# oarodriguez/PhD-QMCLib

Measured on AMD Instinct MI355X. Metric: walker-steps/sec, higher is better.
Workload: dtype f64

## Files before the change

### phd_qmclib_amd/csrc/qmc_device.h

```cpp
#pragma once

#include <hip/hip_runtime.h>
#include <stdint.h>

#include "qmc_math.h"

#define QMC_PI 3.141592653589793238462643383279502884

#define QMC_NSEC 32
#define QMC_SEC_COPIES 1024
#define QMC_NDIAG 4
#if defined(QMC_TIMING)
#define QMC_SECTION(name) qmc_stamp(m, qmc_sec_id(name))
#define QMC_SECTION_PHASE(off) qmc_stamp_phase(off)
#elif defined(QMC_CUTS)
#define QMC_SECTION(name)                                                     \
    do {                                                                      \
        if (m.sec_cut == qmc_sec_id(name) + QMC_SEC_OFF)                      \
            __builtin_amdgcn_endpgm();                                        \
    } while (0)
#define QMC_SECTION_PHASE(off) do { } while (0)
#elif defined(QMC_SECTIONS)
#define QMC_SECTION(name) asm volatile("; SECTION " name)
#define QMC_SECTION_PHASE(off) do { } while (0)
// ... 74 lines not shown
    unsigned long long last[4];
    int cur[4], phase[4];
};
__device__ __forceinline__ QmcStampState &qmc_stamp_state()
{
    __shared__ QmcStampState st;
    return st;
}
__device__ __forceinline__ void qmc_stamp_phase(int off)
{
    if ((threadIdx.x & 63) == 0) qmc_stamp_state().phase[threadIdx.x >> 6] = off;
}
__device__ __forceinline__ void qmc_stamp(const DevModel &m, int id)
{
    const unsigned long long t = __builtin_readcyclecounter();
    if ((threadIdx.x & 63) == 0 && m.sec_prof) {
        QmcStampState &st = qmc_stamp_state();
        const int w = threadIdx.x >> 6;
        if (id != 0) {
            const int c = (st.cur[w] & (QMC_NSEC - 1)) +
                          2 * QMC_NSEC * (blockIdx.x & (QMC_SEC_COPIES - 1));
            atomicAdd(&m.sec_prof[c], t - st.last[w]);
            atomicAdd(&m.sec_prof[QMC_NSEC + c], 1ull);
        } else {
            st.phase[w] = 0;
        }
        st.cur[w] = id + st.phase[w];
        st.last[w] = t;
    }
}
#endif

#define OB_DEG 7
#define OB_ROW 16

enum { STREAM_VMC_MOVE = 0, STREAM_VMC_ACCEPT = 1, STREAM_DMC_BRANCH = 2,
       STREAM_DMC_DIFFUSE = 3 };

__device__ __forceinline__ void philox4x32_10(uint32_t (&c)[4], uint32_t k0,
                                              uint32_t k1)
{
#pragma unroll
    for (int r = 0; r < 10; ++r) {
        uint64_t p0 = (uint64_t)0xD2511F53u * c[0];
        uint64_t p1 = (uint64_t)0xCD9E8D57u * c[2];
        uint32_t n0 = (uint32_t)(p1 >> 32) ^ c[1] ^ k0;
        uint32_t n2 = (uint32_t)(p0 >> 32) ^ c[3] ^ k1;
        c[0] = n0; c[1] = (uint32_t)p1; c[2] = n2; c[3] = (uint32_t)p0;
        k0 += 0x9E3779B9u; k1 += 0xBB67AE85u;
    }
}

__device__ __forceinline__ double u53(uint32_t hi, uint32_t lo)
{
    const double a = (double)(hi >> 5);
    const double b = (double)(lo >> 6);
    return fma(a, 0x1p-27, b * 0x1p-53);
}

__device__ __forceinline__ void philox_uniform2(uint64_t seed, uint32_t slot,
                                                uint32_t step, uint32_t index,
                                                uint32_t stream, double &u0,
                                                double &u1)
{
    uint32_t c[4] = { slot, step, index, stream };
    philox4x32_10(c, (uint32_t)seed, (uint32_t)(seed >> 32));
    u0 = u53(c[0], c[1]);
    u1 = u53(c[2], c[3]);
}

__device__ __forceinline__ void philox2x32_10(uint32_t &c0, uint32_t &c1,
                                              uint32_t k)
{
#pragma unroll
    for (int r = 0; r < 10; ++r) {
        const uint64_t p = (uint64_t)0xD256D193u * c0;
        const uint32_t n0 = (uint32_t)(p >> 32) ^ k ^ c1;
        c1 = (uint32_t)p;
        c0 = n0;
        k += 0x9E3779B9u;
    }
}

__device__ __forceinline__ void vmc_move_block(uint64_t seed, uint32_t slot,
                                               uint32_t step, uint32_t index,
                                               uint32_t &w0, uint32_t &w1)
{
    uint32_t key = (uint32_t)seed ^ ((uint32_t)(seed >> 32) * 0x85EBCA6Bu);
    key += (step >> 26) * 0x632BE5ABu + (slot >> 28) * 0xC2B2AE35u;
    w0 = ((step & 0x3FFFFFFu) << 6) | ((slot >> 22) & 0x3Fu);
    w1 = ((slot & 0x3FFFFFu) << 10) | (index & 0x3FFu);
    philox2x32_10(w0, w1, key);
}

__device__ __forceinline__ double vmc_move_unit(uint32_t w0)
{
    return fma((double)w0, 0x1p-32, 0x1p-33 - 0.5);
}

__device__ __forceinline__ void normal2_from_uniforms(double u0, double u1,
                                                      double &g0, double &g1)
{
    double r = fast_sqrt(fmax(-2.0 * log_pos(1.0 - u0), 1e-300));
    double s, c;
    sincos_halfpi(4.0 * u1, s, c);
    g0 = r * c;
    g1 = r * s;
}

__device__ __forceinline__ void philox_normal2(uint64_t seed, uint32_t slot,
                                               uint32_t step, uint32_t index,
                                               uint32_t stream, double &g0,
                                               double &g1)
{
    double u0, u1;
    philox_uniform2(seed, slot, step, index, stream, u0, u1);
    normal2_from_uniforms(u0, u1, g0, g1);
}

__device__ __forceinline__ void normal2_from_words(uint32_t w0, uint32_t w1,
                                                   double &g0, double &g1)
{
    const double u0 = fma((double)w0, 0x1p-32, 0x1p-33);
    const double u1 = fma((double)w1, 0x1p-32, 0x1p-33);
    const double r = fast_sqrt(-2.0 * log_pos(u0));
    double s, c;
    sincos_halfpi(4.0 * u1, s, c);
    g0 = r * c;
    g1 = r * s;
}

__device__ __forceinline__ void dmc_normal2(uint64_t seed, uint32_t slot,
                                            uint32_t step2, uint32_t index,
                                            double &g0, double &g1)
{
    uint32_t key = (uint32_t)seed ^ ((uint32_t)(seed >> 32) * 0x85EBCA6Bu);
    key += 0x27D4EB2Fu;
    key += (step2 >> 26) * 0x632BE5ABu + (slot >> 28) * 0xC2B2AE35u;
    uint32_t w0 = ((step2 & 0x3FFFFFFu) << 6) | ((slot >> 22) & 0x3Fu);
    uint32_t w1 = ((slot & 0x3FFFFFu) << 10) | (index & 0x3FFu);
    philox2x32_10(w0, w1, key);
    normal2_from_words(w0, w1, g0, g1);
}

__device__ __forceinline__ double wrap_box(double z, double L)
{
    double zw = (z < 0.0) ? z + L : (z >= L) ? z - L : z;
    const bool far = z < -L || z >= 2.0 * L;
    if (__builtin_expect(__ballot(far) != 0ull, 0)) {
        const double r = fma(-L, floor(z / L), z);
        zw = far ? (r < 0.0 ? r + L : r) : zw;
    }
    return zw;
}

template <int G, int P>
struct SlotMap {
    static constexpr bool CONSECUTIVE = (G == 64) && (P >= 2);
};

template <int G, bool PAD>
__device__ __forceinline__ int lanes_in_use(const DevModel &m)
{
    return PAD ? m.ge : G;
}

template <int G, int P, bool PAD>
__device__ __forceinline__ int walker_n(const DevModel &m)
{
    return PAD ? m.n : G * P;
}

template <int G, int P, bool PAD>
__device__ __forceinline__ int lane_particle(const DevModel &m, int gl, int p)
{
    if (SlotMap<G, P>::CONSECUTIVE) return P * gl + p;
    if (!PAD) return gl + G * p;
    const int ge = m.ge;
    return gl < ge ? gl + ge * p : m.n;
}

template <int N>
__device__ __forceinline__ double row_ror_f64(double v)
{
    const int lo = __builtin_amdgcn_update_dpp(0, __double2loint(v), 0x120 + N,
                                               0xf, 0xf, false);
    const int hi = __builtin_amdgcn_update_dpp(0, __double2hiint(v), 0x120 + N,
                                               0xf, 0xf, false);
    return __hiloint2double(hi, lo);
}

template <int G>
__device__ __forceinline__ double group_sum(double v)
{
    static_assert(G >= 16, "lane groups are 16, 32 or 64 lanes");
    v += row_ror_f64<8>(v);
    v += row_ror_f64<4>(v);
    v += row_ror_f64<2>(v);
    v += row_ror_f64<1>(v);
#pragma unroll
    for (int m = 16; m < G; m <<= 1)
        v += __shfl_xor(v, m, 64);
    return v;
}

__device__ __forceinline__ double wave_sum_mfma(double v)
{
    const double r = __builtin_amdgcn_mfma_f64_4x4x4f64(v, 1.0, 0.0, 0, 0, 0);
    double t = __builtin_amdgcn_mfma_f64_4x4x4f64(r, 1.0, 0.0, 0, 0, 0);
    t += row_ror_f64<4>(t);
    t += row_ror_f64<8>(t);
    return t;
}

template <int G, int P>
__device__ __forceinline__ void resort_step(double (&z)[P], int (&lab)[P],
                                            int gl, unsigned parity, int n,
                                            double L, double half_L,
                                            int ge = G)
{
    const int lane = threadIdx.x & 63, base = lane - gl;
    int pg = (parity & 1u) ? ((gl & 1) ? gl + 1 : gl - 1) : (gl ^ 1);
    const bool wrap_hi = pg >= ge, wrap_lo = pg < 0;
    if (wrap_hi) pg = 0;
    if (wrap_lo) pg = ge - 1;
    double z0[P]; int l0[P];
#pragma unroll
    for (int a = 0; a < P; ++a) { z0[a] = z[a]; l0[a] = lab[a]; }
#pragma unroll
    for (int a = 0; a < P; ++a) {
        const int want = wrap_hi ? (a + 1) % P : (wrap_lo ? (a + P - 1) % P : a);
        double zp = 0.0; int lp = 0;
#pragma unroll
        for (int b = 0; b < P; ++b) {
            double zz = __shfl(z0[b], base + pg, 64);
            int ll = __shfl(l0[b], base + pg, 64);
            if (b == want) { zp = zz; lp = ll; }
        }
        const bool valid = gl < ge && (gl + ge * a) < n &&
                           (pg + ge * want) < n;
        const bool lower = wrap_hi ? true : (wrap_lo ? false : gl < pg);
        double d = lower ? zp - z0[a] : z0[a] - zp;
        if (d > half_L) d -= L;
        if (d < -half_L) d += L;
        if (valid && d < 0.0) { z[a] = zp; lab[a] = lp; }
    }
}

template <int G>
__device__ __forceinline__ void resort_linear(double &z, int &lab, int gl,
                                              unsigned parity, int ge)
{
    const int lane = threadIdx.x & 63, base = lane - gl;
    const int pg = (parity & 1u) ? ((gl & 1) ? gl + 1 : gl - 1) : (gl ^ 1);
    const bool has = gl < ge && pg >= 0 && pg < ge;
    const int src = base + (has ? pg : gl);
    const double zp = __shfl(z, src, 64);
    const int lp = __shfl(lab, src, 64);
    const bool take = has && ((gl < pg) ? zp < z : zp > z);
    if (take) { z = zp; lab = lp; }
}

template <int G>
__device__ __forceinline__ int group_ror1_b32(int x)
{
    static_assert(G == 64 || G == 16, "a DPP rotation exists for 16 and 64 lanes");
    if (G == 64) return __builtin_amdgcn_update_dpp(x, x, 0x13C, 0xf, 0xf, false);
    return __builtin_amdgcn_update_dpp(x, x, 0x121, 0xf, 0xf, false);
}
template <int G>
__device__ __forceinline__ double group_ror1(double v)
{
    return __hiloint2double(group_ror1_b32<G>(__double2hiint(v)),
                            group_ror1_b32<G>(__double2loint(v)));
}
template <int G>
__device__ __forceinline__ float group_ror1(float v)
{
    return __int_as_float(group_ror1_b32<G>(__float_as_int(v)));
}

__device__ __forceinline__ double readlane_f64(double v, int lane)
{
    const int lo = __builtin_amdgcn_readlane(__double2loint(v), lane);
    const int hi = __builtin_amdgcn_readlane(__double2hiint(v), lane);
    return __hiloint2double(hi, lo);
}

__device__ __forceinline__ void anchor_seam(double &z, int &lab,
                                            int ge )
{
    const int lane = threadIdx.x & 63;
    const double z0 = readlane_f64(z, 0), zl = readlane_f64(z, ge - 1);
    if (zl < z0) {
        const double z1 = readlane_f64(z, 1), zl1 = readlane_f64(z, ge - 2);
        int src = lane;
        if (zl < z1) {
            if (lane < ge) src = lane == 0 ? ge - 1 : lane - 1;
        } else if (z0 > zl1) {
            if (lane < ge) src = lane == ge - 1 ? 0 : lane + 1;
        }
        z = __shfl(z, src, 64);
        lab = __shfl(lab, src, 64);
    }
}

// ... 969 lines not shown
```

### phd_qmclib_amd/csrc/qmc_kernels.h

```cpp
#pragma once

#include "qmc_device.h"
#include "qmc_sorted64.h"
#include "qmc_sorted128.h"

static constexpr int BLOCK = 256;

static constexpr int BLOCK64 = 64;
template <int G>
struct WalkBlock {
    static constexpr int N = (G == 64) ? BLOCK64 : BLOCK;
};

template <int GPB>
__device__ __forceinline__ long long walker_of_block(unsigned b, int grp)
{
    if (GPB == 1)
        return ((long long)(b >> 7) << 7) + ((b & 7u) << 4) + ((b & 127u) >> 3);
    return (long long)b * GPB + grp;
}

template <int G, int P, bool PAD, bool ZC, bool DMC = false>
struct StepLds {
    static constexpr int NROWS =
        DMC ? SortedCot<false, true, false>::ROWS : 5;
    static constexpr int SORTED =
        (G == 64 && P == 2 && !ZC)   ? NROWS * SortedRows<128>::ROW
        : (G == 64 && P == 1 && !ZC) ? NROWS * SortedRows<64>::ROW
                                     : 0;
    static constexpr int GENERAL = GroupLds<G, P, ZC>::DOUBLES;
    static constexpr int DOUBLES = SORTED > GENERAL ? SORTED : GENERAL;
};

__device__ __forceinline__ long long qmc_uniform(long long v)
{
    const int lo = __builtin_amdgcn_readfirstlane((int)v);
    const int hi = __builtin_amdgcn_readfirstlane((int)(v >> 32));
    return ((long long)hi << 32) | (unsigned int)lo;
}
__device__ __forceinline__ int qmc_opaque(int v)
{
    asm volatile("" : "+v"(v));
    return v;
}
__device__ __forceinline__ double qmc_uniform_f64(double v)
{
    return __longlong_as_double(qmc_uniform(__double_as_longlong(v)));
}
__device__ __forceinline__ double qmc_lane_f64(double v, int k)
{
    const long long b = __double_as_longlong(v);
    const int lo = __builtin_amdgcn_readlane((int)b, k);
    const int hi = __builtin_amdgcn_readlane((int)(b >> 32), k);
    return __longlong_as_double(((long long)hi << 32) | (unsigned int)lo);
}

__device__ __forceinline__ double vmc_accept_thresholds(uint64_t seed,
                                                        uint32_t slot,
                                                        uint32_t step0, int lane,
                                                        int n)
{
    uint32_t m0, m1, hi, lo;
    vmc_move_block(seed, slot, step0 + (uint32_t)lane, 0u, m0, hi);
    vmc_move_block(seed, slot, step0 + (uint32_t)lane, n == 1 ? 0u : 1u, m1, lo);
    const double ua = u53(hi, lo);
    const double h = 0.5 * log_pos(ua);
    return ua <= 0.0 ? __builtin_nan("") : h;
}

static constexpr int LB_P1 = 7;
static constexpr int LB_DMC_P2 = 5;
static constexpr int LB_VMC_P2 = 4;
constexpr int lb_waves(int G, int P, bool ZC, int p2)
{
    return (G == 64 && P == 1) ? LB_P1 : (G == 64 && P == 2 && !ZC) ? p2 : 1;
}


template <int P>
struct DmcSpare {
    static constexpr bool ON = P == 1;
};

static constexpr int RESORT_EVERY = 4;

struct EvalArgs {
    const double *pos;
    double *wf, *energy;
    double *ith, *drift;
    long long nconf;
};

template <int G, int P, bool PAD, bool ZC, typename R = double>
__global__ void __launch_bounds__(WalkBlock<G>::N, lb_waves(G, P, ZC, 1))
evaluate_kernel(const DevModel *__restrict__ mp, EvalArgs a)
{
    const DevModel &m = *mp;
    [[maybe_unused]] constexpr int QMC_SEC_OFF = 0;
    QMC_SECTION("top");
    extern __shared__ double smem[];
    constexpr int GPB = WalkBlock<G>::N / G;
    const int grp = threadIdx.x / G, gl = threadIdx.x % G;
    double *lds = smem + (size_t)grp * GroupLds<G, P, ZC>::DOUBLES;
    const long long w = walker_of_block<GPB>(blockIdx.x, grp);
    const bool active = w < a.nconf;
    if (GPB == 1 && !active) return;
    const long long wr = active ? w : 0;
    const int n = walker_n<G, P, PAD>(m);
    double z[P], z1[P], F[P], ei[P], E, wf;
#pragma unroll
    for (int p = 0; p < P; ++p) {
        int i = lane_particle<G, P, PAD>(m, gl, p);
        z1[p] = (i < n) ? a.pos[wr * n + i] : 0.0;
        z[p] = wrap_box(z1[p], m.L);
    }
    eval_walker<G, P, PAD, true, true, ZC, R>(m, z, z1, gl, lds, F, ei, E, wf);
    if (!active) return;
#pragma unroll
    for (int p = 0; p < P; ++p) {
        int i = lane_particle<G, P, PAD>(m, gl, p);
        if (i < n) {
            if (a.ith) a.ith[w * n + i] = ei[p];
            if (a.drift) a.drift[w * n + i] = F[p];
        }
    }
    if (gl == 0) {
        if (a.wf) a.wf[w] = wf;
        if (a.energy) a.energy[w] = E;
    }
}

struct PrepArgs {
    const double *pos;
    double *drift, *energy;
    long long nconf;
};

template <int G, int P, bool PAD, bool ZC, typename R = double>
__global__ void __launch_bounds__(WalkBlock<G>::N, lb_waves(G, P, ZC, 1))
prepare_kernel(const DevModel *__restrict__ mp, PrepArgs a)
{
    const DevModel &m = *mp;
    [[maybe_unused]] constexpr int QMC_SEC_OFF = 0;
    QMC_SECTION("top");
    extern __shared__ double smem[];
    constexpr int GPB = WalkBlock<G>::N / G;
    const int grp = threadIdx.x / G, gl = threadIdx.x % G;
    double *lds = smem + (size_t)grp * GroupLds<G, P, ZC>::DOUBLES;
    const long long w = walker_of_block<GPB>(blockIdx.x, grp);
    const bool active = w < a.nconf;
    if (GPB == 1 && !active) return;
    const long long wr = active ? w : 0;
    const int n = walker_n<G, P, PAD>(m);
    double z[P], z1[P], F[P], ei[P], E, wf;
#pragma unroll
    for (int p = 0; p < P; ++p) {
        int i = lane_particle<G, P, PAD>(m, gl, p);
        z1[p] = (i < n) ? a.pos[wr * n + i] : 0.0;
        z[p] = wrap_box(z1[p], m.L);
    }
    eval_walker<G, P, PAD, false, false, ZC, R>(m, z, z1, gl, lds, F, ei, E,
                                                wf);
    if (!active) return;
#pragma unroll
    for (int p = 0; p < P; ++p) {
        int i = lane_particle<G, P, PAD>(m, gl, p);
        if (i < n) a.drift[w * n + i] = F[p];
    }
    if (gl == 0) a.energy[w] = E;
}

struct alignas(64) VmcRec {
    double wf;
    double ecarry;
    double sum_e, sum_e2;
    long long n_acc;
    long long spare[3];
};
static_assert(sizeof(VmcRec) == 64, "one record = 8 eight-byte words");
typedef unsigned int VmcRecWords __attribute__((ext_vector_type(16)));
#define QMC_CONST __attribute__((address_space(4)))
__device__ __forceinline__ double vmc_rec_word(const VmcRecWords &r, int k)
{
    return __hiloint2double((int)r[2 * k + 1], (int)r[2 * k]);
}

struct VmcArgs {
    double *pos;
    unsigned short *label;
    VmcRec *rec;
    double *ser_wf, *ser_e;
    unsigned char *ser_stat;
    double *ser_pos;
    const double *tape;
    long long tape_steps;
    long long tape_idx;
    long long W;
    long long y;
    unsigned int nsteps;
    int forced;
    int reset_sums;
    int gaussian;
    unsigned int step;
    unsigned int chain0;
    unsigned long long seed;
    double move_spread;
};

template <int G, int P, bool ZC>
struct VmcFused {
    static constexpr bool ON = G == 64 && !ZC && (P == 1 || P == 2);
};

template <int G, int P, bool PAD, bool ZC, bool LEAN, typename R = double,
          bool STEADY = false>
__global__ void __launch_bounds__(WalkBlock<G>::N, lb_waves(G, P, ZC, LB_VMC_P2))
vmc_step_kernel(const DevModel *__restrict__ mp, VmcArgs a)
{
    static_assert(LEAN || !STEADY, "the steady variant is a LEAN kernel");
    const DevModel &m = *mp;
    [[maybe_unused]] constexpr int QMC_SEC_OFF = 0;
    QMC_SECTION("top");
    extern __shared__ double smem[];
    constexpr int GPB = WalkBlock<G>::N / G;
    const int grp = threadIdx.x / G, gl = threadIdx.x % G;
    static_assert(StepLds<G, P, PAD, ZC>::DOUBLES >= GroupLds<G, P, ZC>::DOUBLES,
                  "eval_walker is the fallback on the same LDS region");
    double *lds = smem + (size_t)grp * StepLds<G, P, PAD, ZC>::DOUBLES;
    const long long w = walker_of_block<GPB>(blockIdx.x, grp);
    const bool active = w < a.W;
    if (GPB == 1 && !active) return;
    const long long wr = active ? w : 0;
    const int n = walker_n<G, P, PAD>(m);
    const unsigned int slot = a.chain0 + (unsigned int)wr;
    const bool forced = !STEADY && a.forced != 0;
    const bool reset_sums = !STEADY && a.reset_sums != 0;

    const long long wl = (G == 64) ? qmc_uniform(wr) : wr;
    double wf_cur, e_cur, se = 0.0, se2 = 0.0;
    long long na = 0;
    if constexpr (G == 64) {
        const VmcRecWords r = *(const QMC_CONST VmcRecWords *)(a.rec + wl);
        wf_cur = vmc_rec_word(r, 0);
        e_cur = vmc_rec_word(r, 1);
        se = vmc_rec_word(r, 2);
        se2 = vmc_rec_word(r, 3);
        na = __double_as_longlong(vmc_rec_word(r, 4));
        if (reset_sums) { se = 0.0; se2 = 0.0; na = 0; }
    } else {
        wf_cur = a.rec[wl].wf;
        e_cur = a.rec[wl].ecarry;
    }

    constexpr bool FUSED = STEADY && VmcFused<G, P, ZC>::ON;
    double zc[P];
    int labc[P];
    [[maybe_unused]] double thr = 0.0;
    if constexpr (FUSED) {
#pragma unroll
        for (int p = 0; p < P; ++p) {
            int i = lane_particle<G, P, PAD>(m, gl, p);
            zc[p] = (i < n) ? a.pos[wr * n + i] : 0.0;
            labc[p] = (i < n) ? (int)a.label[wr * n + i] : i;
        }
    }
    bool any_acc = false;
    const unsigned int nst = FUSED ? a.nsteps : 1u;
    bool acc = false;
    [[maybe_unused]] const int gl_top = gl;
    for (unsigned int s = 0; s < nst; ++s) {
    const unsigned int step = a.step + s;
    constexpr bool REDERIVE = FUSED && (P != 1 || PAD);
    const int gl = REDERIVE ? qmc_opaque(gl_top) : gl_top;
    if constexpr (FUSED) {
        if ((s & 63u) == 0u)
            thr = vmc_accept_thresholds(a.seed, slot, step, gl, n);
    }
    QMC_SECTION("load+philox+wrap");
    double zn[P];
    int labn[P];
    double ua = 1.0;
    unsigned int aw0 = 0u, aw1 = 0u;
    bool has0 = false, has1 = false;
    bool outside = false;
#pragma unroll
    for (int p = 0; p < P; ++p) {
        int i = lane_particle<G, P, PAD>(m, gl, p);
        double zp;
        if constexpr (FUSED) {
            zp = zc[p];
            labn[p] = labc[p];
        } else {
            zp = (i < n) ? a.pos[wr * n + i] : 0.0;
            labn[p] = (i < n) ? (int)a.label[wr * n + i] : i;
        }
        const unsigned li = (unsigned)labn[p];
        double d = 0.0;
        if (!forced && i < n) {
            if (!LEAN && a.tape) {
                double tv = a.tape[(wr * a.tape_steps + a.tape_idx) * (n + 1) + li];
                d = a.gaussian ? a.move_spread * tv
                               : (tv - 0.5) * a.move_spread;
            } else if (!LEAN && a.gaussian) {
                double g0, g1;
                philox_normal2(a.seed, slot, step, li, STREAM_VMC_MOVE, g0,
                               g1);
                d = a.move_spread * g0;
            } else {
                uint32_t w0, w1;
                vmc_move_block(a.seed, slot, step, li, w0, w1);
                d = vmc_move_unit(w0) * a.move_spread;
                if constexpr (!FUSED) {
                    if (li == 0u) { aw0 = w1; has0 = true; }
                    if (li == 1u || n == 1) { aw1 = w1; has1 = true; }
                }
            }
        }
        double zs;
        {
#pragma clang fp contract(off)
            zs = zp + d;
        }
        zn[p] = wrap_box(zs, m.L);
        if (forced) outside = outside || zn[p] != zp;
    }
    QMC_SECTION("resort");
    constexpr bool S64 = G == 64 && P == 1 && !ZC;
    constexpr bool S128 = G == 64 && P == 2 && !ZC;
    bool fast = false;
    if (forced)
        outside = __builtin_amdgcn_ballot_w64(outside) != 0ull;
    if constexpr (S64) {
        fast = !m.is_ideal && !outside &&
               sort_lanes64(zn[0], labn[0], gl, PAD ? n : 64) &&
               (PAD ? far_partner_ok_ring(m, zn[0], gl, n)
                    : far_partner_ok64(m, zn[0], gl));
    } else if constexpr (S128) {
        fast = !m.is_ideal && !outside && (!PAD || (n & 1) == 0) &&
               sort_rows128(zn, labn, gl, PAD ? n / 2 : 64) &&
               (PAD ? far_partner_ok_ring128(m, zn, gl, n / 2)
                    : far_partner_ok128(m, zn, gl));
    }
    if constexpr (S64 || S128) {
        if (!fast && !m.is_ideal && gl == 0 && active)
            atomicAdd(m.diag, 1ull);
    } else if constexpr (G == 64 && P == 1) {
        if (!forced) {
            anchor_seam(zn[0], labn[0], n);
            if ((a.step % RESORT_EVERY) == 0)
                resort_linear<G>(zn[0], labn[0], gl,
                                 a.step / RESORT_EVERY, n);
        }
    } else if constexpr (SlotMap<G, P>::CONSECUTIVE) {
        if (!forced) {
            anchor_seam_rows<P>(zn, labn, n);
            if ((a.step % RESORT_EVERY) == 0)
                resort_linear_rows<P>(zn, labn, gl, a.step / RESORT_EVERY, n);
        }
    } else if (!forced && (a.step % RESORT_EVERY) == 0)
        resort_step<G, P>(zn, labn, gl, a.step / RESORT_EVERY, n, m.L,
                          m.half_L, lanes_in_use<G, PAD>(m));
    constexpr bool TWO_PASS = G == 64;
    double F[P], ei[P], e_new = 0.0, wf_new;
    if (S64 && fast) {
        if constexpr (S64)
            eval_sorted64<R, true, false, false, PAD>(
                m, zn[0], gl, lds, F[0], e_new, wf_new);
    } else if (S128 && fast) {
        if constexpr (S128)
            eval_sorted128<R, true, false, false, PAD>(m, zn, gl, lds, F,
                                                       e_new, wf_new);
    } else {
        double z1[P];
#pragma unroll
        for (int p = 0; p < P; ++p) {
            int i = lane_particle<G, P, PAD>(m, gl, p);
            z1[p] = (outside && i < n) ? a.pos[wr * n + i] : zn[p];
        }
        if constexpr (TWO_PASS)
            eval_walker<G, P, PAD, true, false, ZC, R, false, false>(
                m, zn, z1, gl, lds, F, ei, e_new, wf_new);
        else
            eval_walker<G, P, PAD, true, false, ZC, R>(m, zn, z1, gl, lds, F,
                                                       ei, e_new, wf_new);
    }
    QMC_SECTION("metropolis+store");
    if (FUSED) {
    } else if (!forced) {
        if (!LEAN && a.tape) {
            ua = a.tape[(wr * a.tape_steps + a.tape_idx) * (n + 1) + n];
        } else if (!LEAN && a.gaussian) {
            double u1;
            philox_uniform2(a.seed, slot, step, 0u, STREAM_VMC_ACCEPT, ua,
                            u1);
        } else {
            const unsigned long long bal0 = __ballot(has0);
            const unsigned long long bal1 = __ballot(has1);
            unsigned int hi, lo;
            if (G == 64) {
                const int src0 = __builtin_amdgcn_readfirstlane(
                    (int)__ffsll((long long)bal0) - 1) & 63;
                const int src1 = __builtin_amdgcn_readfirstlane(
                    (int)__ffsll((long long)bal1) - 1) & 63;
                hi = (unsigned)__builtin_amdgcn_readlane((int)aw0, src0);
                lo = (unsigned)__builtin_amdgcn_readlane((int)aw1, src1);
            } else {
                const int base = (threadIdx.x & 63) - gl;
                const unsigned long long gmask = (1ull << (G & 63)) - 1ull;
                const int src0 = base + ((__ffsll((long long)((bal0 >> base) &
                                                              gmask)) - 1) & (G - 1));
                const int src1 = base + ((__ffsll((long long)((bal1 >> base) &
                                                              gmask)) - 1) & (G - 1));
                hi = (unsigned)__shfl((int)aw0, src0, 64);
                lo = (unsigned)__shfl((int)aw1, src1, 64);
            }
            ua = u53(hi, lo);
        }
    }
    if (!active) return;
    if constexpr (FUSED) {
        const double w0 = qmc_uniform_f64(wf_new);
        const double h = qmc_lane_f64(thr, (int)(s & 63u));
        acc = h != h || w0 > wf_cur;
        if (!acc) acc = w0 > h + wf_cur;
        acc = __builtin_amdgcn_readfirstlane((int)acc) != 0;
    } else {
        acc = forced || ua <= 0.0 || wf_new > wf_cur;
        if (!acc) acc = wf_new > 0.5 * log_pos(ua) + wf_cur;
        if (G == 64) acc = __builtin_amdgcn_readfirstlane((int)acc) != 0;
    }
    if (acc) {
        if constexpr (TWO_PASS) {
            QMC_SECTION("energy_pass");
            QMC_SECTION_PHASE(QMC_NSEC / 2);
            double wf_unused;
            if (S64 && fast) {
                if constexpr (S64)
                    eval_sorted64<R, false, true, true, PAD>(
                        m, zn[0], gl, lds, F[0], e_new, wf_unused);
            } else if (S128 && fast) {
                if constexpr (S128)
                    eval_sorted128<R, false, true, true, PAD>(
                        m, zn, gl, lds, F, e_new, wf_unused);
            } else {
                double z1[P];
#pragma unroll
                for (int p = 0; p < P; ++p) {
                    int i = lane_particle<G, P, PAD>(m, gl, p);
                    z1[p] = (outside && i < n) ? a.pos[wr * n + i] : zn[p];
                }
                eval_walker<G, P, PAD, false, false, ZC, R, true, true>(
                    m, zn, z1, gl, lds, F, ei, e_new, wf_unused);
            }
            QMC_SECTION_PHASE(0);
            QMC_SECTION("store");
        }
        if constexpr (FUSED) {
#pragma unroll
            for (int p = 0; p < P; ++p) {
                zc[p] = zn[p];
                labc[p] = labn[p];
            }
            any_acc = true;
        } else {
#pragma unroll
            for (int p = 0; p < P; ++p) {
                int i = lane_particle<G, P, PAD>(m, gl, p);
                if (i < n && !forced) {
                    a.pos[w * n + i] = zn[p];
                    a.label[w * n + i] = (unsigned short)labn[p];
                }
            }
        }
        if (!FUSED) {
            wf_cur = wf_new;
            e_cur = e_new;
        }
    }
    if constexpr (FUSED) {
        if (acc) {
            wf_cur = qmc_uniform_f64(wf_new);
            const double e2 = qmc_lane_f64(e_new, 2);
            const double e3 = qmc_lane_f64(e_new, 3);
            e_cur = qmc_lane_f64(e_new, 1);
            se = se + e2;
            se2 = fma(e3, e3, se2);
            na = na + 1;
        } else {
            se = se + e_cur;
            se2 = fma(e_cur, e_cur, se2);
        }
        se = qmc_uniform_f64(se);
        se2 = qmc_uniform_f64(se2);
        continue;
    }
    if (!LEAN && a.ser_pos) {
#pragma unroll
        for (int p = 0; p < P; ++p) {
            int i = lane_particle<G, P, PAD>(m, gl, p);
            if (i < n) {
                const bool moved = acc && !forced;
                const int lb = moved ? labn[p] : (int)a.label[w * n + i];
                a.ser_pos[(a.y * a.W + w) * n + lb] =
                    moved ? zn[p] : a.pos[w * n + i];
            }
        }
    }
    if (G == 64) {
        const double sum1 = se + e_cur;
        const double sum2 = fma(e_cur, e_cur, se2);
        const long long na1 = qmc_uniform(na + (acc ? 1 : 0));
        double v = __longlong_as_double((gl == 4) ? na1 : 0ll);
        v = (gl == 0) ? wf_cur : v;
        v = (gl == 1) ? e_cur : v;
        v = (gl == 2) ? sum1 : v;
        v = (gl == 3) ? sum2 : v;
        if (gl < 8) reinterpret_cast<double *>(a.rec + wl)[gl] = v;
    }
    if (gl == 0) {
        if (G != 64) {
            VmcRec *r = a.rec + w;
            if (!reset_sums) { se = r->sum_e; se2 = r->sum_e2; na = r->n_acc; }
            r->wf = wf_cur;
            r->ecarry = e_cur;
            r->sum_e = se + e_cur;
            r->sum_e2 = fma(e_cur, e_cur, se2);
            r->n_acc = na + (acc ? 1 : 0);
        }
        if (!LEAN) {
            if (a.ser_wf) a.ser_wf[a.y * a.W + w] = wf_cur;
            if (a.ser_e) a.ser_e[a.y * a.W + w] = e_cur;
            if (a.ser_stat) a.ser_stat[a.y * a.W + w] = acc ? 1 : 0;
        }
    }
    }
    if constexpr (FUSED) {
        QMC_SECTION("fused_store");
        if (any_acc) {
#pragma unroll
            for (int p = 0; p < P; ++p) {
                int i = lane_particle<G, P, PAD>(m, gl, p);
                if (i < n) {
                    a.pos[w * n + i] = zc[p];
                    a.label[w * n + i] = (unsigned short)labc[p];
                }
            }
        }
        double v = __longlong_as_double((gl == 4) ? qmc_uniform(na) : 0ll);
        v = (gl == 0) ? wf_cur : v;
        v = (gl == 1) ? e_cur : v;
        v = (gl == 2) ? se : v;
        v = (gl == 3) ? se2 : v;
        if (gl < 8) reinterpret_cast<double *>(a.rec + wl)[gl] = v;
    }
    QMC_SECTION("end");
}

struct DmcCtl {
    long long prev_nw;
    long long nw;
    double ref_energy;
    double total_energy, total_weight;
    double e_t, w_t;
    long long spare_nw;
    unsigned int step;
    unsigned int pad;
};

struct EvolveArgs {
    const double *ppos, *pdrift, *penergy;
    double *cpos, *cdrift, *cenergy, *cweight;
    const unsigned short *plabel;
    unsigned short *clabel;
    double *eslot;
    const long long *ref;
// ... 138 lines not shown
```

### phd_qmclib_amd/csrc/qmcwalk.hip

```cpp
#include "qmc_inst.h"
#include "qmc_kernels_misc.h"
#include "qmc_obdm.h"
#include "qmc_pairdist.h"
#include "qmc_tripledist.h"
#include "qmc_energy_parts.h"
#include "qmc_renyi.h"
#include "qmc_renyi_region.h"
#include "qmc_partent.h"
#include "qmc_obdm_grid.h"
#include "qmc_cmdiff.h"
#include "qmc_isf.h"
#include "qmc_site.h"
#include "qmc_vmc_sweep.h"
#include "../../include/qmcwalk.h"
#include "qmc_probe.h"

#include <cmath>
#include <cstdio>
#include <cstdlib>
#include <cstring>
#include <algorithm>
#include <memory>
#include <string>
#include <utility>
// ... 102 lines not shown
        if (on) (void)hipEventRecord(e->prof_ev[e->prof_used], e->stream);
    }
    ~ProfScope()
    {
        if (on) {
            (void)hipEventRecord(e->prof_ev[e->prof_used + 1], e->stream);
            e->prof_used += 2;
        }
    }
};


static int pick_shape(int n, int &G, int &P, bool &pad)
{
    if (n < 1) return 1;
    if (const char *env = getenv("QMCWALK_SHAPE")) {
        int g = 0, p = 0;
        if (sscanf(env, "%d,%d", &g, &p) == 2 && n <= g * p) {
#define QMC_LEGAL(sg, sp) || (g == sg && p == sp)
            if (false QMC_FOR_ALL_SHAPES(QMC_LEGAL)) {
                G = g; P = p; pad = (n != G * P);
                return 0;
            }
#undef QMC_LEGAL
        }
    }
    if (n <= 16) { G = 16; P = 1; }
    else if (n <= 32) { G = 16; P = 2; }
    else if (n <= 64) { G = 64; P = 1; }
    else if (n <= 128) { G = 64; P = 2; }
    else if (n <= 256) { G = 64; P = 4; }
    else if (n <= 512) { G = 64; P = 8; }
    else return 1;
    pad = (n != G * P);
    return 0;
}

#define QMC_EXTERN_TU(name) QMC_TU_##name(extern)
QMC_FOR_ALL_TUS(QMC_EXTERN_TU)
#undef QMC_EXTERN_TU
QMC_TU_SWEEP(extern)
QMC_TU_EPARTS(extern)

static constexpr int MASK_FROM_P = 4;

template <template <int, int, bool, bool> class L, typename... A>
static int dispatch_shape(const qmc_engine *e, A &&...args)
{
    const bool zc = e->dm.zclass != 0;
#define QMC_CASE(g, p)                                                        \
    if (e->G == g && e->P == p) {                                             \
        if (p >= MASK_FROM_P || e->pad) {                                     \
            if (zc) return L<g, p, true, true>::run(e, args...);              \
            return L<g, p, true, false>::run(e, args...);                     \
        }                                                                     \
        if constexpr (p < MASK_FROM_P) {                                      \
            if (zc) return L<g, p, false, true>::run(e, args...);             \
            return L<g, p, false, false>::run(e, args...);                    \
        }                                                                     \
    }
    QMC_FOR_ALL_SHAPES(QMC_CASE)
#undef QMC_CASE
    return fail("unsupported boson_number");
}

template <int G, int P, bool ZC>
static size_t lds_bytes()
{
    return (size_t)(WalkBlock<G>::N / G) * GroupLds<G, P, ZC>::DOUBLES *
           sizeof(double);
}

template <int G, int P, bool PAD, bool ZC, bool DMC = false>
static size_t step_lds_bytes()
{
    return (size_t)(WalkBlock<G>::N / G) *
           StepLds<G, P, PAD, ZC, DMC>::DOUBLES * sizeof(double);
}

template <typename K>
static void allow_lds(K kernel, size_t bytes)
{
    if (bytes > 48 * 1024)
        (void)hipFuncSetAttribute((const void *)kernel,
                                  hipFuncAttributeMaxDynamicSharedMemorySize,
                                  (int)bytes);
}

template <int G>
static unsigned grid_for(long long nwalkers)
{
    const long long gpb = WalkBlock<G>::N / G;
    long long blocks = (nwalkers + gpb - 1) / gpb;
    if (gpb == 1) blocks = (blocks + 127) / 128 * 128;
    return (unsigned)blocks;
}

template <int G, typename A>
static int launch_walkers(const qmc_engine *e,
                          void (*kernel)(const DevModel *, A), size_t lds,
                          long long nwalkers, const A &a)
{
    allow_lds(kernel, lds);
    hipLaunchKernelGGL(kernel, dim3(grid_for<G>(nwalkers)),
                       dim3(WalkBlock<G>::N), lds, e->stream, e->dm_dev, a);
    HIP_TRY(hipGetLastError());
    return 0;
}

template <int G, bool ZC>
static constexpr bool has_fast() { return G == 64 && !ZC; }

template <int G, bool ZC, typename F>
static int with_pair_type(const qmc_engine *e, F f)
{
    if constexpr (has_fast<G, ZC>())
        if (e->fast) return f(float{});
    return f(double{});
}

template <int G, int P, bool PAD, bool ZC>
struct LaunchEval {
    static int run(const qmc_engine *e, const EvalArgs &a)
    {
        if (a.nconf <= 0) return 0;
        return with_pair_type<G, ZC>(e, [&](auto r) {
            return launch_walkers<G>(
                e, evaluate_kernel<G, P, PAD, ZC, decltype(r)>,
                lds_bytes<G, P, ZC>(), a.nconf, a);
        });
    }
};

template <int G, int P, bool PAD, bool ZC>
struct LaunchPrep {
    static int run(const qmc_engine *e, const PrepArgs &a)
    {
        if (a.nconf <= 0) return 0;
        return with_pair_type<G, ZC>(e, [&](auto r) {
            return launch_walkers<G>(
                e, prepare_kernel<G, P, PAD, ZC, decltype(r)>,
                lds_bytes<G, P, ZC>(), a.nconf, a);
        });
    }
};

template <int G, int P, bool PAD, bool ZC>
struct LaunchVmc {
    static int run(const qmc_engine *e, const VmcArgs &a, long long *ran)
    {
        const size_t lds = step_lds_bytes<G, P, PAD, ZC>();
        const bool lean = !a.tape && !a.gaussian && !a.ser_wf && !a.ser_e &&
                          !a.ser_stat && !a.ser_pos;
        const bool steady = lean && !a.forced && !a.reset_sums;
        *ran = (steady && VmcFused<G, P, ZC>::ON) ? (long long)a.nsteps : 1;
        ProfScope prof(e);
        return with_pair_type<G, ZC>(e, [&](auto r) {
            using R = decltype(r);
            auto kernel = steady ? vmc_step_kernel<G, P, PAD, ZC, true, R, true>
                          : lean ? vmc_step_kernel<G, P, PAD, ZC, true, R, false>
                                 : vmc_step_kernel<G, P, PAD, ZC, false, R, false>;
            return launch_walkers<G>(e, kernel, lds, a.W, a);
        });
    }
};

template <int G, int P, bool PAD, bool ZC>
struct LaunchSweep {
    static int run(const qmc_engine *e, const VmcArgs &a)
    {
        ProfScope prof(e);
        const size_t lds = (size_t)(WalkBlock<G>::N / G) *
                           SweepLds<G, P, PAD, ZC>::DOUBLES * sizeof(double);
        return launch_walkers<G>(e, vmc_sweep_kernel<G, P, PAD, ZC>, lds, a.W,
                                 a);
    }
};

template <int G, int P, bool PAD, bool ZC>
struct LaunchEvolve {
    static int run(const qmc_engine *e, const EvolveArgs &a)
    {
        ProfScope prof(e);
        return with_pair_type<G, ZC>(e, [&](auto r) {
            return launch_walkers<G>(
                e, dmc_evolve_kernel<G, P, PAD, ZC, decltype(r)>,
                step_lds_bytes<G, P, PAD, ZC, true>(), a.maxw, a);
        });
    }
};

template <int G, int P, bool PAD, bool ZC>
struct LaunchEvolve2 {
    static int run(const qmc_engine *e, const EvolveArgs &a)
    {
        ProfScope prof(e);
        const size_t lds = (size_t)(WalkBlock<G>::N / G) *
                           Step2Lds<G, P, PAD, ZC>::DOUBLES * sizeof(double);
        return with_pair_type<G, ZC>(e, [&](auto r) {
            return launch_walkers<G>(
                e, dmc_evolve2_kernel<G, P, PAD, ZC, decltype(r)>, lds, a.maxw,
                a);
        });
    }
};

static void build_dev_model(const qmc_model_params &p, DevModel &d)
{
    memset(&d, 0, sizeof(d));
    d.n = (int)p.boson_number;
    d.is_free = p.is_free != 0;
    d.is_ideal = p.is_ideal != 0;
    d.defects_sep = (int)(p.defects_sep > 0 ? p.defects_sep : 1);
    d.L = p.supercell_size;
    d.half_L = 0.5 * d.L;
    d.rm = fabs(p.tbf_contact_cutoff);
    d.L_minus_rm = d.L - d.rm;
    d.two_over_L = 2.0 / d.L;
    d.k2_2pi = p.param_k2 * (2.0 / QMC_PI);
    d.k2 = p.param_k2;
    d.k2sq = d.k2 * d.k2;
    double phi = p.param_k2 * p.param_r_off;
    d.cphi = cos(phi);
    d.sphi = sin(phi);
    d.sec_cut = -1;
    d.am_cphi = fabs(p.param_am) * d.cphi;
    d.am_sphi = fabs(p.param_am) * d.sphi;
    d.m_k2cphi = -d.k2 * d.cphi;
    d.k2sphi = d.k2 * d.sphi;
    double th = p.param_k2 * d.L;
    d.cth = cos(th);
    d.sth = fabs(sin(th));
    d.sth_sign = sin(th) < 0.0 ? (int)0x80000000u : 0;
    d.sth_signed = sin(th);
    d.sp_ok = (!d.is_ideal && th > 0.0 && th < QMC_PI - 1e-9 &&
               d.rm < d.half_L) ? 1 : 0;
    d.sp_xlo = -d.k2 * sin(d.k2 * d.rm - phi);
    d.sp_xhi = d.k2 * sin(phi);
    d.sp_cos = cos(d.k2 * d.rm);
    {
        const double ang[4] = { -phi, phi, phi - th, th - phi };
        for (int v = 0; v < 4; ++v) {
            d.var_cos[v] = cos(ang[v]);
            d.var_sin[v] = sin(ang[v]);
        }
        d.m_k2 = -d.k2;
    }
    d.sin_rm = (d.rm >= d.half_L) ? 1.0 : sin(QMC_PI * d.rm / d.L);
    d.zclass = d.rm > 0.45 * d.L;
    double pi_L = QMC_PI / d.L;
    d.a_long = pi_L * p.param_beta;
    d.b_long = pi_L * pi_L * p.param_beta;
    d.a_long_sq = d.a_long * d.a_long;
    d.m_k2_over_a = d.a_long != 0.0 ? -d.k2 / d.a_long : 0.0;
    d.m_a_over_k2 = d.k2 != 0.0 ? -d.a_long / d.k2 : 0.0;
    d.beta = p.param_beta;
    d.inv_beta = p.param_beta != 0.0 ? 1.0 / p.param_beta : 0.0;
    d.one_minus_beta = 1.0 - p.param_beta;
    d.log_am = log(fabs(p.param_am));
    d.z_a = 1.0 / (1.0 + p.lattice_ratio);
    d.z_b = p.lattice_ratio / (1.0 + p.lattice_ratio);
    d.k1 = p.param_k1;
    d.k1_2pi = p.param_k1 * (2.0 / QMC_PI);
    d.kp1 = p.param_kp1;
    d.e0 = p.param_e0;
    d.v0 = p.lattice_depth;
    d.v0d = p.defect_magnitude;
    d.uniform_barrier = (d.defects_sep == 1 || d.v0d == d.v0) ? 1 : 0;
    d.v_barrier = (d.defects_sep == 1) ? d.v0d : d.v0;
    d.k1_half = 0.5 * p.param_k1;
    d.v0_minus_e0 = p.lattice_depth - p.param_e0;
    if (!d.is_free) {
        double sh = sinh(0.5 * sqrt(d.v0 - d.e0) * d.z_b);
        d.cf = sqrt(1 + d.v0 / d.e0 * sh * sh);
    } else {
        d.cf = 1.0;
    }
}

static void ob_exact(const DevModel &d, long double zc, bool barrier,
                     long double &ldz, long double &logf)
{
    if (barrier) {
        const long double x = (long double)d.kp1 *
                              (zc - 1.0L + 0.5L * (long double)d.z_b);
        ldz = (long double)d.kp1 * tanhl(x);
        logf = logl(coshl(x));
    } else {
        const long double x = (long double)d.k1 *
                              (zc - 0.5L * (long double)d.z_a);
        ldz = -(long double)d.k1 * tanl(x);
        logf = logl((long double)d.cf * cosl(x));
    }
}

template <int DEG, typename F>
static void ob_fit(F f, long double a, long double h, double *coef)
{
    constexpr int K = DEG + 1;
    long double A[K][K + 1];
    for (int j = 0; j < K; ++j) {
        const long double t = 0.5L * (1.0L + cosl(3.14159265358979323846264338L *
                                                  (2 * j + 1) / (2.0L * K)));
        long double pw = 1.0L;
        for (int k = 0; k < K; ++k) { A[j][k] = pw; pw *= t; }
        A[j][K] = f(a + h * t);
    }
    for (int c = 0; c < K; ++c) {
// ... 3174 lines not shown
```

Before: 771.0 million.

## Halve threshold Philox calls, skip far-wrap ballot, and fuse reset-sums VMC launches

The accept-threshold generator now runs one Philox block per lane and swaps halves across the wave with permlane32_swap, instead of two blocks per lane. Thresholds are regenerated every 32 steps rather than every 64. When every particle starts inside the box and the move spread is bounded, the fused loop uses a simple one-step wrap with no far-check ballot. The fused steady kernel now also accepts reset_sums launches, so those run multi-step instead of one step per launch. This adds a wave-uniform branch on the wrap path and depends on the threshold stream mapping staying equivalent.

Result: faster. 779.6 million, median of 6 (+1.1%).

```diff
diff --git a/phd_qmclib_amd/csrc/qmc_device.h b/phd_qmclib_amd/csrc/qmc_device.h
--- a/phd_qmclib_amd/csrc/qmc_device.h
+++ b/phd_qmclib_amd/csrc/qmc_device.h
@@ -250,6 +250,11 @@
         zw = far ? (r < 0.0 ? r + L : r) : zw;
     }
     return zw;
+}
+
+__device__ __forceinline__ double wrap_box_near(double z, double L)
+{
+    return (z < 0.0) ? z + L : (z >= L) ? z - L : z;
 }
 
 template <int G, int P>
diff --git a/phd_qmclib_amd/csrc/qmc_kernels.h b/phd_qmclib_amd/csrc/qmc_kernels.h
--- a/phd_qmclib_amd/csrc/qmc_kernels.h
+++ b/phd_qmclib_amd/csrc/qmc_kernels.h
@@ -55,14 +55,18 @@
     return __longlong_as_double(((long long)hi << 32) | (unsigned int)lo);
 }
 
+static constexpr unsigned int VMC_THR_YIELDS = 32u;
 __device__ __forceinline__ double vmc_accept_thresholds(uint64_t seed,
                                                         uint32_t slot,
                                                         uint32_t step0, int lane,
                                                         int n)
 {
-    uint32_t m0, m1, hi, lo;
-    vmc_move_block(seed, slot, step0 + (uint32_t)lane, 0u, m0, hi);
-    vmc_move_block(seed, slot, step0 + (uint32_t)lane, n == 1 ? 0u : 1u, m1, lo);
+    const bool upper = lane >= 32;
+    uint32_t mv, own;
+    vmc_move_block(seed, slot, step0 + (uint32_t)(lane & 31),
+                   (upper && n != 1) ? 1u : 0u, mv, own);
+    const auto sw = __builtin_amdgcn_permlane32_swap(own, own, false, false);
+    const uint32_t hi = sw[0], lo = sw[1];
     const double ua = u53(hi, lo);
     const double h = 0.5 * log_pos(ua);
     return ua <= 0.0 ? __builtin_nan("") : h;
@@ -234,7 +238,8 @@
     const int n = walker_n<G, P, PAD>(m);
     const unsigned int slot = a.chain0 + (unsigned int)wr;
     const bool forced = !STEADY && a.forced != 0;
-    const bool reset_sums = !STEADY && a.reset_sums != 0;
+    const bool reset_sums =
+        (!STEADY || VmcFused<G, P, ZC>::ON) && a.reset_sums != 0;
 
     const long long wl = (G == 64) ? qmc_uniform(wr) : wr;
     double wf_cur, e_cur, se = 0.0, se2 = 0.0;
@@ -264,6 +269,15 @@
             labc[p] = (i < n) ? (int)a.label[wr * n + i] : i;
         }
     }
+    [[maybe_unused]] bool near = false;
+    if constexpr (FUSED) {
+        bool inside = true;
+#pragma unroll
+        for (int p = 0; p < P; ++p)
+            inside = inside && zc[p] >= 0.0 && zc[p] < m.L;
+        near = __builtin_amdgcn_ballot_w64(!inside) == 0ull &&
+               a.move_spread >= 0.0 && a.move_spread <= 2.0 * m.L;
+    }
     bool any_acc = false;
     const unsigned int nst = FUSED ? a.nsteps : 1u;
     bool acc = false;
@@ -273,7 +287,7 @@
     constexpr bool REDERIVE = FUSED && (P != 1 || PAD);
     const int gl = REDERIVE ? qmc_opaque(gl_top) : gl_top;
     if constexpr (FUSED) {
-        if ((s & 63u) == 0u)
+        if ((s & (VMC_THR_YIELDS - 1u)) == 0u)
             thr = vmc_accept_thresholds(a.seed, slot, step, gl, n);
     }
     QMC_SECTION("load+philox+wrap");
@@ -321,7 +335,7 @@
 #pragma clang fp contract(off)
             zs = zp + d;
         }
-        zn[p] = wrap_box(zs, m.L);
+        zn[p] = (FUSED && near) ? wrap_box_near(zs, m.L) : wrap_box(zs, m.L);
         if (forced) outside = outside || zn[p] != zp;
     }
     QMC_SECTION("resort");
@@ -420,7 +434,7 @@
     if (!active) return;
     if constexpr (FUSED) {
         const double w0 = qmc_uniform_f64(wf_new);
-        const double h = qmc_lane_f64(thr, (int)(s & 63u));
+        const double h = qmc_lane_f64(thr, (int)(s & (VMC_THR_YIELDS - 1u)));
         acc = h != h || w0 > wf_cur;
         if (!acc) acc = w0 > h + wf_cur;
         acc = __builtin_amdgcn_readfirstlane((int)acc) != 0;
diff --git a/phd_qmclib_amd/csrc/qmcwalk.hip b/phd_qmclib_amd/csrc/qmcwalk.hip
--- a/phd_qmclib_amd/csrc/qmcwalk.hip
+++ b/phd_qmclib_amd/csrc/qmcwalk.hip
@@ -278,8 +278,9 @@
         const size_t lds = step_lds_bytes<G, P, PAD, ZC>();
         const bool lean = !a.tape && !a.gaussian && !a.ser_wf && !a.ser_e &&
                           !a.ser_stat && !a.ser_pos;
-        const bool steady = lean && !a.forced && !a.reset_sums;
-        *ran = (steady && VmcFused<G, P, ZC>::ON) ? (long long)a.nsteps : 1;
+        constexpr bool FUSED = VmcFused<G, P, ZC>::ON;
+        const bool steady = lean && !a.forced && (FUSED || !a.reset_sums);
+        *ran = (steady && FUSED) ? (long long)a.nsteps : 1;
         ProfScope prof(e);
         return with_pair_type<G, ZC>(e, [&](auto r) {
             using R = decltype(r);
```
